# berkeley-hipie/HIPIE

Measured on AMD Instinct MI355X. Metric: images/sec @1024x1024 ViT-H bs=8 (single-image inference hot path: box, class and mask logits), higher is better.
Workload: dtype f16x3 (split-fp16 operands, fp32 accumulate: fp32-class); 1 GPU; BASELINE.json configs[2]: vit_huge, 1024x1024, batch 8 per GPU, 80 class prompts (L=194), detection; global_batch=8, parallelism=dp1, precision_policy=split, launch=eager

## Files before the change

### hipie_amd/csrc/gemm.hip

```cpp
#include "gemm_tile.h"

namespace hipie {

template <typename T>
__global__ __launch_bounds__(256) void to_hl8_kernel(const T* __restrict__ x, f16_t* __restrict__ out, long rows, int K, long ldx, long ldo,
                                                     float scale) {
  const long gid = (long)blockIdx.x * 256 + threadIdx.x;
  const int gpr = K / 8;
  if (gid >= rows * gpr) return;
  const long r = gid / gpr;
  const int g = (int)(gid - r * gpr);
  const T* src = x + r * ldx + 8 * g;
  f16x8 h, l;
#pragma unroll
  for (int e = 0; e < 8; ++e) {
    f16_t hh, ll;
    hl_split((float)src[e] * scale, hh, ll);
    h[e] = hh;
    l[e] = ll;
  }
  f16_t* dst = out + r * ldo + 16 * g;
  *reinterpret_cast<f16x8*>(dst) = h;
  *reinterpret_cast<f16x8*>(dst + 8) = l;
}
// ... 23 lines not shown
  __syncthreads();
  for (int u = tid; u < kTrCols * (kTrRows / 8); u += 256) {
    const int g = u % (kTrRows / 8), c = u / (kTrRows / 8);
    const long m = r0 + 8 * g;
    if (c0 + c >= C || m >= rows_p) continue;
    f16x8 h, l;
#pragma unroll
    for (int e = 0; e < 8; ++e) {
      f16_t hh, ll;
      hl_split(tile[8 * g + e][c] * scale, hh, ll);
      h[e] = hh;
      l[e] = ll;
    }
    f16_t* dst = out + (long)(c0 + c) * ldo + 2 * m;
    *reinterpret_cast<f16x8*>(dst) = h;
    *reinterpret_cast<f16x8*>(dst + 8) = l;
  }
}

}

using namespace hipie;

namespace hipie {
int launch_gemm_k256(const void* X, long ldx_b, int x_f32, const void* W, long ldw_b, const float* bias, float* out, long ldo, int M, int N,
                     hipStream_t st);
}

static inline bool gemm_mfma16() {
  const char* e = study_env("HIPIE_GEMM_MFMA");
  return e ? atoi(e) == 16 : true;
}

static int gemm_impl(const void* A, int64_t lda, const void* W, int64_t ldw, const float* bias, const float* resid, int64_t ldr,
                     void* out, int64_t ldo, const int32_t* out_row, const int32_t* a_row, int64_t a_rows, int M, int N, int K, int in_fmt,
                     int out_fmt, int act, float alpha, float oscale, void* stream, const float* alpha_dev = nullptr) {
  HIPIE_REQUIRE(A && W && out, "gemm: null pointer");
  HIPIE_REQUIRE(in_fmt == HIPIE_F16 || in_fmt == HIPIE_HL8 || in_fmt == HIPIE_F32, "gemm: operand format %d (HIPIE_F16 | HIPIE_HL8 | HIPIE_F32)",
                in_fmt);
  HIPIE_REQUIRE(out_fmt == HIPIE_F32 || out_fmt == HIPIE_F16 || out_fmt == HIPIE_HL8, "gemm: output format %d", out_fmt);
  HIPIE_REQUIRE(act >= 0 && act <= 3, "gemm: activation %d (0 none, 1 gelu, 2 relu, 3 quick-gelu)", act);
  HIPIE_REQUIRE(M > 0 && N > 0 && K > 0 && N % 8 == 0, "gemm: M=%d N=%d K=%d (N must be a multiple of 8)", M, N, K);
  const bool a_f32 = in_fmt == HIPIE_F32;
  const bool split = in_fmt == HIPIE_HL8 || a_f32;
  if (a_f32) lda *= 2;
  const int kq = split ? 32 : 64;
  HIPIE_REQUIRE(K % kq == 0, "gemm: K=%d must be a multiple of %d", K, kq);
  const int epr = split ? 2 * K : K;
  HIPIE_TRY(gm_check_operands("gemm", lda, ldw, epr, 320));
  HIPIE_TRY(gm_check_out("gemm", ldo, out_fmt, N));
  HIPIE_TRY(gm_check_resid("gemm", resid, ldr, N));
  HIPIE_TRY(gm_check_aligned("gemm", {A, W, out, bias, resid}));
  GemmParams p;
  gm_set_operands(p, A, lda, W, ldw, M, N, K, kq);
  p.bias = bias; p.resid = resid; p.ldr = ldr; p.out = (char*)out; p.ldo = ldo; p.out_row = out_row; p.a_row = a_row;
  p.out_fmt = out_fmt; p.act = act; p.alpha = alpha; p.oscale = oscale; p.alpha_dev = alpha_dev;
  hipStream_t st = (hipStream_t)stream;
  static const int k256_mode = [] { const char* e = study_env("HIPIE_GEMM_K256"); return e ? atoi(e) : 2; }();
  const bool k256_on = k256_mode == 1 || (k256_mode == 2 && N >= 384);
  if (k256_on && split && K == 256 && out_fmt == HIPIE_F32 && act == 0 && resid == nullptr && out_row == nullptr && a_row == nullptr &&
      alpha == 1.f && oscale == 1.f && alpha_dev == nullptr && N % 32 == 0 && M >= 8192 && ldw * 2 == 1024 && (long)M * p.lda_b < (1L << 32))
    return launch_gemm_k256(A, p.lda_b, a_f32 ? 1 : 0, W, p.ldw_b, bias, (float*)out, ldo, M, N, st);
  const bool wide = (N % 320 == 0);
  static const int small_on = [] { const char* e = study_env("HIPIE_GEMM_SMALL"); return e ? atoi(e) : 1; }();
  static const long small_tiles = [] { const char* e = study_env("HIPIE_GEMM_SMALL_MAXTILES"); return e ? atol(e) : 96L; }();
  const bool small_ok = small_on && (long)((M + 255) / 256) * ((N + (wide ? 319 : 255)) / (wide ? 320 : 256)) < small_tiles;
#ifdef HIPIE_GEMM_VARIANTS
  { const char* e = study_env("HIPIE_GEMM_VARIANT"); const int v = e ? atoi(e) : 0;
    if (split && wide && v == 1) return launch_gemm<320, true, 1>(p, st);
    if (split && wide && v == 3) return launch_gemm<320, true, 3>(p, st); }
  { const char* e = study_env("HIPIE_GEMM_VARIANT"); if (e) p.variant = atoi(e); }
  p.prio_mode = gemm2_prio();
  if (split && gemm2_mode() == 4) {
    const bool w160 = (N % 160 == 0);
    if (a_f32) return w160 ? launch_gemm4<5, 2>(p, st) : launch_gemm4<4, 2>(p, st);
    return w160 ? launch_gemm4<5, 0>(p, st) : launch_gemm4<4, 0>(p, st);
  }
  if (split && gemm2_mode() == 2) {
    const bool w160 = (N % 160 == 0);
    if (a_f32) return w160 ? launch_gemm3<5, 2>(p, st) : launch_gemm3<4, 2>(p, st);
    return w160 ? launch_gemm3<5, 0>(p, st) : launch_gemm3<4, 0>(p, st);
  }
  if (split && gemm2_mode() == 1) {
    const bool w160 = (N % 160 == 0);
    if (a_f32) return w160 ? launch_gemm2<5, 2>(p, st) : launch_gemm2<4, 2>(p, st);
    return w160 ? launch_gemm2<5, 0>(p, st) : launch_gemm2<4, 0>(p, st);
  }
#endif
  if (split && small_ok && a_row == nullptr) return a_f32 ? launch_gemm_small<2>(p, st) : launch_gemm_small<0>(p, st);
  if (split && wide && gemm_mfma16()) return a_f32 ? launch_gemm<320, true, 2, 16>(p, st) : launch_gemm<320, true, 0, 16>(p, st);
  if (a_f32) return wide ? launch_gemm<320, true, 2>(p, st) : launch_gemm<256, true, 2>(p, st);
  if (split) return wide ? launch_gemm<320, true>(p, st) : launch_gemm<256, true>(p, st);
  return wide ? launch_gemm<320, false>(p, st) : launch_gemm<256, false>(p, st);
}

extern "C" int hipie_gemm(const void* A, int64_t lda, const void* W, int64_t ldw, const float* bias, const float* resid, int64_t ldr,
                          void* out, int64_t ldo, const int32_t* out_row, int M, int N, int K, int in_fmt, int out_fmt, int act, float alpha,
                          float oscale, void* stream) {
  return gemm_impl(A, lda, W, ldw, bias, resid, ldr, out, ldo, out_row, nullptr, 0, M, N, K, in_fmt, out_fmt, act, alpha, oscale, stream);
}

extern "C" int hipie_gemm_scaled(const void* A, int64_t lda, const void* W, int64_t ldw, const float* bias, const float* resid, int64_t ldr,
                                 void* out, int64_t ldo, const int32_t* out_row, int M, int N, int K, int in_fmt, int out_fmt, int act, float alpha,
                                 float oscale, const float* alpha_dev, void* stream) {
  HIPIE_REQUIRE(((uintptr_t)alpha_dev % 4) == 0, "gemm_scaled: alpha_dev must be 4-byte aligned");
  return gemm_impl(A, lda, W, ldw, bias, resid, ldr, out, ldo, out_row, nullptr, 0, M, N, K, in_fmt, out_fmt, act, alpha, oscale, stream, alpha_dev);
}

extern "C" int hipie_gemm_gather(const void* A, int64_t lda, int64_t a_rows, const int32_t* a_row, const void* W, int64_t ldw, const float* bias,
                                 const float* resid, int64_t ldr, void* out, int64_t ldo, const int32_t* out_row, int M, int N, int K, int in_fmt,
                                 int out_fmt, int act, float alpha, float oscale, void* stream) {
  HIPIE_REQUIRE(a_row != nullptr && a_rows > 0, "gemm_gather: a_row map / operand row count missing");
  HIPIE_REQUIRE(in_fmt == HIPIE_HL8 || in_fmt == HIPIE_F32, "gemm_gather: split operands only (HIPIE_HL8 | HIPIE_F32 rows)");
  HIPIE_REQUIRE((long)a_rows * lda * (in_fmt == HIPIE_F32 ? 4 : 2) < (1L << 32), "gemm_gather: the gathered operand must stay below 4 GiB");
  return gemm_impl(A, lda, W, ldw, bias, resid, ldr, out, ldo, out_row, a_row, a_rows, M, N, K, in_fmt, out_fmt, act, alpha, oscale, stream);
}

extern "C" int hipie_gemm_batched(const void* A, int64_t lda, int64_t a_outer, int64_t a_inner, const void* W, int64_t ldw, int64_t w_outer,
                                  int64_t w_inner, void* out, int64_t ldo, int64_t o_outer, int64_t o_inner, int n_outer, int n_inner, int M,
                                  int N, int K, int out_fmt, float alpha, void* stream) {
  HIPIE_REQUIRE(A && W && out, "gemm_batched: null pointer");
  HIPIE_REQUIRE(out_fmt == HIPIE_F32 || out_fmt == HIPIE_HL8, "gemm_batched: output format %d (HIPIE_F32 | HIPIE_HL8)", out_fmt);
  HIPIE_REQUIRE(M > 0 && N > 0 && K > 0 && N % 8 == 0 && K % 32 == 0, "gemm_batched: M=%d N=%d K=%d (N %% 8, K %% 32)", M, N, K);
// ... 126 lines not shown
```

### hipie_amd/csrc/gemm_k256.hip

```cpp
#include <stdlib.h>

#include "common.h"
#include "mfma.h"
#include "wave.h"

namespace hipie {

struct TKParams {
  const char* X; const char* W; const float* bias; float* out;
  long ldx_b, ldw_b, ldo;
  int M, N;
};

constexpr int TK_K = 256, TK_C = 32;
constexpr int TK_TILE = TK_C * TK_K * 4;

template <bool XF32>
__global__ __launch_bounds__(256, 2) void gemm_k256_kernel(const TKParams p) {
  typedef f16_t T;
  typedef Mfma32<T>::frag frag;
  constexpr int KS = TK_K / 16;
  extern __shared__ __attribute__((aligned(1024))) char smem[];

  const int tid = threadIdx.x, lane = tid & 63;
  const int wave = __builtin_amdgcn_readfirstlane(tid >> 6);
  const int li = lane & 31, hi = lane >> 5;
  const int m = blockIdx.x * 128 + wave * 32 + li;
  const int mc = min(m, p.M - 1);
  const int nch = p.N / TK_C;

  unsigned int dv[8];
#pragma unroll
  for (int q = 0; q < 8; ++q) {
    const int i = wave + 4 * q;
    dv[q] = (unsigned int)((long)i * p.ldw_b + 16 * (lane ^ (i & 15)));
  }
  const unsigned int lds0 = (unsigned int)reinterpret_cast<uintptr_t>((__attribute__((address_space(3))) char*)smem);
  auto dma_chunk = [&](const int c, const int buf, const int q) __attribute__((always_inline)) {
    const int i = wave + 4 * q;
    dma16(p.W + (long)c * TK_C * p.ldw_b, dv[q], __builtin_amdgcn_readfirstlane(lds0 + (unsigned int)(buf * TK_TILE + 1024 * i)));
  };

  frag xh[KS], xl[KS];
  {
    const int m0w = blockIdx.x * 128 + wave * 32;
    const unsigned int xslice = lds0 + (unsigned int)(wave * 16384);
    const char* xs = smem + wave * 16384 + li * 512;
    unsigned int xv[16];
#pragma unroll
    for (int j = 0; j < 16; ++j) {
// ... 9 lines not shown
#pragma unroll
      for (int ksl = 0; ksl < KS / 2; ++ksl) {
        const int ks = half * (KS / 2) + ksl;
        const int u = 2 * (2 * ksl + hi);
        const frag a = *reinterpret_cast<const frag*>(xs + 16 * (u ^ (li & 15)));
        const frag b = *reinterpret_cast<const frag*>(xs + 16 * ((u + 1) ^ (li & 15)));
        if (XF32) {
          const f32x4 fa = __builtin_bit_cast(f32x4, a), fb = __builtin_bit_cast(f32x4, b);
          const float v[8] = {fa[0], fa[1], fa[2], fa[3], fb[0], fb[1], fb[2], fb[3]};
#pragma unroll
          for (int e = 0; e < 8; ++e) {
            T h, l;
            hl_split(v[e], h, l);
            xh[ks][e] = h;
            xl[ks][e] = l;
          }
        } else {
          xh[ks] = a;
          xl[ks] = b;
        }
      }
    }
    __builtin_amdgcn_s_waitcnt(lgkmcnt0);
    __syncthreads();
  }
#pragma unroll
  for (int q = 0; q < 8; ++q) dma_chunk(0, 0, q);

  const int wrow = li * 1024, wsw = li & 15;
  float* orow = p.out + (long)mc * p.ldo + 4 * hi;
  float4 prev[4];
#pragma unroll
  for (int g = 0; g < 4; ++g) prev[g] = make_float4(0.f, 0.f, 0.f, 0.f);

  for (int c = 0; c < nch; ++c) {
    const int buf = c & 1;
    __builtin_amdgcn_s_waitcnt(vmcnt(0));
    __syncthreads();
    if (c > 0 && m < p.M) {
#pragma unroll
      for (int g = 0; g < 4; ++g) *reinterpret_cast<float4*>(orow + 32 * (c - 1) + 8 * g) = prev[g];
    }
    const char* bs = smem + buf * TK_TILE;
    const bool more = c + 1 < nch;
    f32x16 h0, h1;
#pragma unroll
    for (int r = 0; r < 16; ++r) { h0[r] = 0.f; h1[r] = 0.f; }
#pragma unroll
    for (int ks = 0; ks < KS; ks += 2) {
      const frag ah0 = *reinterpret_cast<const frag*>(bs + wrow + 16 * ((2 * (2 * ks + hi)) ^ wsw));
      const frag al0 = *reinterpret_cast<const frag*>(bs + wrow + 16 * ((2 * (2 * ks + hi) + 1) ^ wsw));
      const frag ah1 = *reinterpret_cast<const frag*>(bs + wrow + 16 * ((2 * (2 * ks + 2 + hi)) ^ wsw));
      const frag al1 = *reinterpret_cast<const frag*>(bs + wrow + 16 * ((2 * (2 * ks + 2 + hi) + 1) ^ wsw));
      h0 = Mfma32<T>::mma(al0, xh[ks], h0);
      h1 = Mfma32<T>::mma(al1, xh[ks + 1], h1);
      h0 = Mfma32<T>::mma(ah0, xl[ks], h0);
      h1 = Mfma32<T>::mma(ah1, xl[ks + 1], h1);
      h0 = Mfma32<T>::mma(ah0, xh[ks], h0);
      h1 = Mfma32<T>::mma(ah1, xh[ks + 1], h1);
      if (more) dma_chunk(c + 1, buf ^ 1, ks >> 1);
    }
#pragma unroll
    for (int g = 0; g < 4; ++g) {
      float4 b4 = make_float4(0.f, 0.f, 0.f, 0.f);
      if (p.bias) b4 = *reinterpret_cast<const float4*>(p.bias + 32 * c + 8 * g + 4 * hi);
      prev[g] = make_float4(h0[4 * g] + h1[4 * g] + b4.x, h0[4 * g + 1] + h1[4 * g + 1] + b4.y, h0[4 * g + 2] + h1[4 * g + 2] + b4.z,
                            h0[4 * g + 3] + h1[4 * g + 3] + b4.w);
    }
  }
  if (m < p.M) {
#pragma unroll
    for (int g = 0; g < 4; ++g) *reinterpret_cast<float4*>(orow + 32 * (nch - 1) + 8 * g) = prev[g];
  }
}

int launch_gemm_k256(const void* X, long ldx_b, int x_f32, const void* W, long ldw_b, const float* bias, float* out, long ldo, int M, int N,
                     hipStream_t st) {
  TKParams p;
  p.X = (const char*)X; p.W = (const char*)W; p.bias = bias; p.out = out;
  p.ldx_b = ldx_b; p.ldw_b = ldw_b; p.ldo = ldo;
  p.M = M; p.N = N;
  const size_t lds = (size_t)2 * TK_TILE;
  static LdsLimit limit[2];
  limit[0].raise((const void*)gemm_k256_kernel<true>, lds);
  limit[1].raise((const void*)gemm_k256_kernel<false>, lds);
  const dim3 grid((unsigned)((M + 127) / 128));
  if (x_f32) hipLaunchKernelGGL(gemm_k256_kernel<true>, grid, dim3(256), lds, st, p);
  else hipLaunchKernelGGL(gemm_k256_kernel<false>, grid, dim3(256), lds, st, p);
  return check_launch("gemm_k256");
}

}
```

### hipie_amd/csrc/gemm_tile.h

```cpp
#pragma once
#include <stdlib.h>

#include <initializer_list>

#include "common.h"
#include "gelu.h"
#include "mfma.h"
#include "wave.h"

namespace hipie {

struct GemmParams {
  const char* A = nullptr; const char* W = nullptr; const float* bias = nullptr; const float* resid = nullptr; char* out = nullptr;
  const int32_t* out_row = nullptr;
  const int32_t* a_row = nullptr;
  long lda_b = 0, ldw_b = 0;
  long ldr = 0, ldo = 0;
  int M = 0, N = 0, K = 0;
  int nkt = 0;
  int tiles_m = 0, tiles_n = 0;
  int group_m = 0;
  int out_fmt = HIPIE_F32, act = 0;
  float alpha = 1.f, oscale = 1.f;
  int nbi = 1;
// ... 98 lines not shown
                           __builtin_bit_cast(unsigned int, v[g][2]), __builtin_bit_cast(unsigned int, v[g][3])};
    } else {
#pragma unroll
      for (int g = 0; g < NG; ++g) {
        unsigned int H0, L0, H1, L1;
        gm_split2(v[g][0], v[g][1], H0, L0);
        gm_split2(v[g][2], v[g][3], H1, L1);
#if defined(__HIP_DEVICE_COMPILE__) && !defined(HIPIE_NO_FMA_MIX)
        asm volatile("s_nop 1" : "+v"(H0), "+v"(L0), "+v"(H1), "+v"(L1));
#endif
        const u32x2 s0 = __builtin_amdgcn_permlane32_swap(H0, L0, false, false);
        const u32x2 s1 = __builtin_amdgcn_permlane32_swap(H1, L1, false, false);
        piece[g] = (u32x4){s0[0], s1[0], s0[1], s1[1]};
      }
    }
    const long rowb = (m * p.ldo) * (ofmt == HIPIE_F32 ? 4 : 2) + (long)nb * 4 + 16 * hi;
#pragma unroll
    for (int g = 0; g < NG; ++g)
      if (mok && nb + 8 * (G0 + g) < p.N) *reinterpret_cast<u32x4*>(p.out + rowb + 32 * (G0 + g)) = piece[g];
  }
}

template <int G0, int NG>
__device__ __forceinline__ void gm_epi_quads(const f32x16& a, const float4* rq, const float* sb, const long m, const bool mok, const int nb,
                                             const int hi, const GemmParams& p, const bool has_res) {
  float x[NG][4];
#pragma unroll
  for (int g = 0; g < NG; ++g)
#pragma unroll
    for (int e = 0; e < 4; ++e) x[g][e] = a[4 * (G0 + g) + e];
  gm_epi_vals<NG>(x, G0, rq, sb, m, mok, nb, hi, p, has_res);
}

__device__ __forceinline__ constexpr int gm_swz16(const int r) { return ((r >> 1) & 3) | (((((r & 15) + 4) >> 3) & 1) << 2); }

__device__ __forceinline__ void gm_epi_vals16(const float (&x)[2][4], const float4* rq, const float* sb, const long m, const bool mok, const int nb,
                                              const int g, const GemmParams& p, const bool has_res) {
  typedef unsigned int u32x2 __attribute__((ext_vector_type(2)));
  typedef unsigned int u32x4 __attribute__((ext_vector_type(4)));
  const float alpha = p.alpha, osc = p.oscale;
  const int act = p.act, ofmt = p.out_fmt;
  float v[2][4];
#pragma unroll
  for (int i = 0; i < 2; ++i) {
    const float4 b4 = *reinterpret_cast<const float4*>(sb + 16 * i + 4 * g);
    v[i][0] = x[i][0] * alpha + b4.x;
    v[i][1] = x[i][1] * alpha + b4.y;
    v[i][2] = x[i][2] * alpha + b4.z;
    v[i][3] = x[i][3] * alpha + b4.w;
  }
  if (act == 1) {
#pragma unroll
    for (int i = 0; i < 2; ++i)
#pragma unroll
      for (int e = 0; e < 4; ++e) v[i][e] = gm_gelu(v[i][e]);
  } else if (act == 2) {
#pragma unroll
    for (int i = 0; i < 2; ++i)
#pragma unroll
      for (int e = 0; e < 4; ++e) v[i][e] = fmaxf(v[i][e], 0.f);
  } else if (act == 3) {
#pragma unroll
    for (int i = 0; i < 2; ++i)
#pragma unroll
      for (int e = 0; e < 4; ++e) v[i][e] = v[i][e] / (1.f + expf(-1.702f * v[i][e]));
  }
// ... 127 lines not shown
#pragma unroll
  for (int t = 0; t < NT; ++t) {
    const int m = m0 + wm * 64 + t * 16 + c;
    orow[t] = (m < p.M) ? (p.out_row != nullptr ? (long)p.out_row[m] : (long)m) : -1;
  }
  float4 rq[2][2];
  auto load_res = [&](const int blk, float4 (&dst)[2]) {
    const int t = blk / (NF / 2), jp = blk % (NF / 2);
#pragma unroll
    for (int i = 0; i < 2; ++i) {
      const int n = n0 + wn * (BN / 2) + jp * 32 + 16 * i + 4 * g;
      dst[i] = (has_res && orow[t] >= 0 && n < p.N) ? *reinterpret_cast<const float4*>(p.resid + orow[t] * p.ldr + n) : make_float4(0.f, 0.f, 0.f, 0.f);
    }
  };
  load_res(0, rq[0]);
#pragma unroll
  for (int t = 0; t < NT; ++t) {
    const long m = orow[t];
#pragma unroll
    for (int jp = 0; jp < NF / 2; ++jp) {
      const int blk = t * (NF / 2) + jp;
      if (blk + 1 < NT * (NF / 2)) load_res(blk + 1, rq[(blk + 1) & 1]);
      const int nb = n0 + wn * (BN / 2) + jp * 32;
      float x[2][4];
#pragma unroll
      for (int i = 0; i < 2; ++i)
#pragma unroll
        for (int e = 0; e < 4; ++e) x[i][e] = acc[2 * jp + i][t][e];
      gm_epi_vals16(x, rq[blk & 1], sbias + (nb - n0), m, m >= 0, nb, g, p, has_res);
    }
  }
}

template <int BN, bool SPLIT, int VAR, int MS = 32>
__global__ __launch_bounds__(512, 2) void gemm_kernel(const GemmParams pin) {
  static_assert(MS == 32 || (MS == 16 && BN == 320 && SPLIT && (VAR == 0 || VAR == 2)),
                "the 16x16x32 form exists for the wide split instances (HL8 and fp32 A rows) only");
  GemmParams p = pin;
  gm_alpha_dev(p);
  int vtile = -1;
  if (VAR == 8) {
    const int nblk = p.tiles_m * p.tiles_n * p.nbi;
    const int id = blockIdx.x, xcd = id & 7, j = id >> 3;
    const int q = nblk >> 3, r = nblk & 7;
    const int v = (xcd < r ? xcd * (q + 1) : r * (q + 1) + (xcd - r) * q) + j;
    const int bo = blockIdx.y, bi = v % p.nbi;
    vtile = v / p.nbi;
    p.A += bo * p.a_bo + bi * p.a_bi;
    p.W += bo * p.w_bo + bi * p.w_bi;
    p.out += bo * p.o_bo + bi * p.o_bi;
    if (p.sm_mask != nullptr) p.sm_mask += (long)bo * p.sm_L;
    if (p.sm_bias != nullptr) p.sm_bias += ((long)bo * p.nbi + bi) * p.N;
  } else if (gridDim.y > 1) {
    const int bo = blockIdx.y / p.nbi, bi = blockIdx.y - bo * p.nbi;
    p.A += bo * p.a_bo + bi * p.a_bi;
    p.W += bo * p.w_bo + bi * p.w_bi;
    p.out += bo * p.o_bo + bi * p.o_bi;
    if (p.sm_mask != nullptr) p.sm_mask += (long)bo * p.sm_L;
    if (p.sm_bias != nullptr) p.sm_bias += (long)blockIdx.y * p.N;
    if (p.resid != nullptr) p.resid += bo * p.r_bo + bi * p.r_bi;
  }
  constexpr int BM = 256;
  constexpr int ROWS = BM + BN;
  constexpr int STAGE = ROWS * 128;
  constexpr int NI = ROWS / 64;
  constexpr int NJ = BN / 64;
  constexpr int KS = SPLIT ? 2 : 4;
  constexpr int SUB = KS * NJ;
  constexpr bool AF32 = VAR == 2 || VAR == 6;
  constexpr bool LNE = VAR == 4 || VAR == 6;
// ... 104 lines not shown
      if (SPLIT) wa[s & 1][1] = *reinterpret_cast<const frag*>(ws + j * 4096 + choff(ks, 1));
    };
    load_x(0);
    load_w(0);
    constexpr int DMA_BY = SPLIT ? 4 : 6;
    constexpr int PER = (NI + DMA_BY - 1) / DMA_BY;
    frag cx[2][2];
#pragma unroll
    for (int s = 0; s < SUB; ++s) {
      const int ks = s / NJ, j = s % NJ;
      if (s + 1 < SUB) {
        if ((s + 1) % NJ == 0) load_x(ks + 1);
        load_w(s + 1);
      }
      if (AF32 && j == 0) {
#pragma unroll
        for (int t = 0; t < 2; ++t) {
          const f32x4 a = __builtin_bit_cast(f32x4, xa[ks & 1][0][t]), b = __builtin_bit_cast(f32x4, xa[ks & 1][1][t]);
#pragma unroll
          for (int e = 0; e < 4; ++e) {
            f16_t hh, ll;
            hl_split(a[e], hh, ll);
            cx[0][t][e] = hh; cx[1][t][e] = ll;
            hl_split(b[e], hh, ll);
            cx[0][t][4 + e] = hh; cx[1][t][4 + e] = ll;
          }
        }
      }
      const frag wh = wa[s & 1][0];
      const frag xh0 = AF32 ? cx[0][0] : xa[ks & 1][0][0], xh1 = AF32 ? cx[0][1] : xa[ks & 1][0][1];
      if (SPLIT) {
        const frag wl = wa[s & 1][1];
        const frag xl0 = AF32 ? cx[1][0] : xa[ks & 1][1][0], xl1 = AF32 ? cx[1][1] : xa[ks & 1][1][1];
        acc[j][0] = Mfma32<f16_t>::mma(wl, xh0, acc[j][0]);
        acc[j][1] = Mfma32<f16_t>::mma(wl, xh1, acc[j][1]);
        acc[j][0] = Mfma32<f16_t>::mma(wh, xl0, acc[j][0]);
        acc[j][1] = Mfma32<f16_t>::mma(wh, xl1, acc[j][1]);
      }
      acc[j][0] = Mfma32<f16_t>::mma(wh, xh0, acc[j][0]);
      acc[j][1] = Mfma32<f16_t>::mma(wh, xh1, acc[j][1]);
      if (more) {
#pragma unroll
        for (int i = s * PER; i < (s + 1) * PER && i < NI; ++i) dma(i, kt + 1, st ^ 1);
      }
    }
    __builtin_amdgcn_s_waitcnt(vmcnt(0));
    __syncthreads();
  }

  bool has_res = p.resid != nullptr;
#ifdef HIPIE_GEMM_VARIANTS
  if (VAR == 1 && p.alpha != 12345.f) return;
#endif
  const int act = p.act, ofmt = p.out_fmt;
  const float alpha = p.alpha, osc = p.oscale;
  float* sbias = reinterpret_cast<float*>(smem);
  if (tid < BN) sbias[tid] = (p.bias != nullptr && n0 + tid < p.N) ? p.bias[n0 + tid] : 0.f;
  if (SPLIT && LNE && BN == 256) {
    float* lg = sbias + 256;
    float* lb = lg + 256;
    float* red = lb + 256;
    if (tid < 256) { lg[tid] = p.ln_g[tid]; lb[tid] = p.ln_b[tid]; }
    __syncthreads();
    float su[2] = {0.f, 0.f};
    f32x4 rr[2][4];
    auto ln_res = [&](const int blk, f32x4 (&dst)[4]) {
      const int t = blk / NJ, j = blk % NJ;
      const int m = min(m0 + wm * 64 + t * 32 + li, p.M - 1);
#pragma unroll
      for (int g = 0; g < 4; ++g) {
        const int n = wn * (BN / 2) + j * 32 + 8 * g + 4 * hi;
        dst[g] = *reinterpret_cast<const f32x4*>(p.resid + (long)m * p.ldr + n);
      }
// ... 34 lines not shown
      for (int j = 0; j < NJ; ++j)
#pragma unroll
        for (int r = 0; r < 16; ++r) { const float d = acc[j][t][r] - mean[t]; q += d * d; }
      sq[t] = q + __shfl_xor(q, 32);
    }
    __syncthreads();
#pragma unroll
    for (int t = 0; t < 2; ++t)
      if (hi == 0) red[wn * 256 + wm * 64 + t * 32 + li] = sq[t];
    __syncthreads();
    float rstd[2];
#pragma unroll
    for (int t = 0; t < 2; ++t) rstd[t] = rsqrtf((sq[t] + red[(wn ^ 1) * 256 + wm * 64 + t * 32 + li]) / 256.f + p.ln_eps);
#pragma unroll
    for (int j = 0; j < NJ; ++j) {
#pragma unroll
      for (int t = 0; t < 2; ++t)
#pragma unroll
        for (int g = 0; g < 4; ++g) {
          const int n = wn * (BN / 2) + j * 32 + 8 * g + 4 * hi;
          const f32x4 g4 = *reinterpret_cast<const f32x4*>(lg + n), b4 = *reinterpret_cast<const f32x4*>(lb + n);
#pragma unroll
          for (int e = 0; e < 4; ++e) acc[j][t][4 * g + e] = (acc[j][t][4 * g + e] - mean[t]) * rstd[t] * g4[e] + b4[e];
        }
#if defined(__HIP_DEVICE_COMPILE__)
      __builtin_amdgcn_sched_barrier(0);
#endif
    }
    __syncthreads();
    if (tid < BN) sbias[tid] = 0.f;
    p.alpha = 1.f; p.act = 0; p.oscale = 1.f; p.out_fmt = HIPIE_F32;
    has_res = false;
  }
  if (SPLIT && (VAR == 0 || VAR == 8) && BN == 256 && p.softmax) {
    float* kb = sbias + 256;
    float* red = kb + 256;
    float* cb = red + 512;
    if (tid < 256) kb[tid] = (tid < p.sm_L && (p.sm_mask == nullptr || p.sm_mask[tid] != 0)) ? 0.f : -INFINITY;
    if (VAR == 8 && tid < 256) cb[tid] = (p.sm_bias != nullptr && tid < p.N) ? p.sm_bias[tid] : 0.f;
    __syncthreads();
    const float cl = p.sm_clamp;
    float mx[2] = {-INFINITY, -INFINITY};
#pragma unroll
    for (int t = 0; t < 2; ++t)
#pragma unroll
      for (int j = 0; j < NJ; ++j)
#pragma unroll
        for (int g = 0; g < 4; ++g) {
          const f32x4 k4 = *reinterpret_cast<const f32x4*>(kb + wn * (BN / 2) + j * 32 + 8 * g + 4 * hi);
          f32x4 c4 = {0.f, 0.f, 0.f, 0.f};
          if (VAR == 8) c4 = *reinterpret_cast<const f32x4*>(cb + wn * (BN / 2) + j * 32 + 8 * g + 4 * hi);
#pragma unroll
          for (int e = 0; e < 4; ++e) {
            float x = acc[j][t][4 * g + e] * p.alpha;
            if (VAR == 8) x += c4[e];
            if (cl > 0.f) x = __builtin_amdgcn_fmed3f(x, -cl, cl);
            x += k4[e];
            acc[j][t][4 * g + e] = x;
            mx[t] = fmaxf(mx[t], x);
          }
        }
#pragma unroll
    for (int t = 0; t < 2; ++t) {
      mx[t] = fmaxf(mx[t], __shfl_xor(mx[t], 32));
      if (hi == 0) red[wn * 256 + wm * 64 + t * 32 + li] = mx[t];
    }
    __syncthreads();
    float sm[2];
#pragma unroll
    for (int t = 0; t < 2; ++t) {
      const float m = fmaxf(mx[t], red[(wn ^ 1) * 256 + wm * 64 + t * 32 + li]);
      const float m2 = (m == -INFINITY) ? 0.f : m * 1.4426950408889634f;
      float su = 0.f;
#pragma unroll
      for (int j = 0; j < NJ; ++j)
#pragma unroll
        for (int r = 0; r < 16; ++r) {
          const float pv = __builtin_amdgcn_exp2f(acc[j][t][r] * 1.4426950408889634f - m2);
          acc[j][t][r] = pv;
          su += pv;
        }
      sm[t] = su + __shfl_xor(su, 32);
    }
    __syncthreads();
#pragma unroll
    for (int t = 0; t < 2; ++t)
      if (hi == 0) red[wn * 256 + wm * 64 + t * 32 + li] = sm[t];
    __syncthreads();
#pragma unroll
    for (int t = 0; t < 2; ++t) {
      const float tot = sm[t] + red[(wn ^ 1) * 256 + wm * 64 + t * 32 + li];
      const float inv = tot > 0.f ? 1.f / tot : 0.f;
#pragma unroll
      for (int j = 0; j < NJ; ++j)
#pragma unroll
        for (int r = 0; r < 16; ++r) acc[j][t][r] *= inv;
    }
    p.alpha = 1.f;
  }
  __syncthreads();
  float4 rq[2][4];
  long orow[2];
#pragma unroll
  for (int t = 0; t < 2; ++t) {
    const int m = m0 + wm * 64 + t * 32 + li;
    orow[t] = (m < p.M) ? (p.out_row != nullptr ? (long)p.out_row[m] : (long)m) : -1;
  }
  auto load_res = [&](const int t, const int j, float4 (&dst)[4]) {
#pragma unroll
    for (int g = 0; g < 4; ++g) {
      const int n = n0 + wn * (BN / 2) + j * 32 + 8 * g + 4 * hi;
      dst[g] = (has_res && orow[t] >= 0 && n < p.N) ? *reinterpret_cast<const float4*>(p.resid + orow[t] * p.ldr + n) : make_float4(0.f, 0.f, 0.f, 0.f);
    }
  };
  const int passes = (LNE && p.out2 != nullptr) ? 2 : 1;
#pragma unroll
  for (int pass = 0; pass < 2; ++pass) {
    if (pass >= passes) break;
    if (pass == 1) { p.out = p.out2; p.ldo = p.ldo2; p.out_fmt = HIPIE_HL8; }
    load_res(0, 0, rq[0]);
#pragma unroll
    for (int t = 0; t < 2; ++t) {
      const long m = orow[t];
      const bool mok = m >= 0;
#pragma unroll
      for (int j = 0; j < NJ; ++j) {
        const int blk = t * NJ + j;
        if (blk + 1 < 2 * NJ) load_res((blk + 1) / NJ, (blk + 1) % NJ, rq[(blk + 1) & 1]);
        const int nb = n0 + wn * (BN / 2) + j * 32;
        gm_epi_quads<0, 4>(acc[j][t], rq[blk & 1], sbias + (nb - n0), m, mok, nb, hi, p, has_res);
#if defined(__HIP_DEVICE_COMPILE__)
        if (LNE) __builtin_amdgcn_sched_barrier(0);
#endif
// ... 103 lines not shown
  if (tid < BN) sbias[tid] = (p.bias != nullptr && n0 + tid < p.N) ? p.bias[n0 + tid] : 0.f;
  __syncthreads();
  const int nb = n0 + wave * 32;
#pragma unroll
  for (int t = 0; t < 2; ++t) {
    const int mm = m0 + t * 32 + li;
    const long m = (mm < p.M) ? (p.out_row != nullptr ? (long)p.out_row[mm] : (long)mm) : -1;
    float4 rq[4];
#pragma unroll
    for (int g = 0; g < 4; ++g) {
      const int n = nb + 8 * g + 4 * hi;
      rq[g] = (has_res && m >= 0 && n < p.N) ? *reinterpret_cast<const float4*>(p.resid + m * p.ldr + n) : make_float4(0.f, 0.f, 0.f, 0.f);
    }
    gm_epi_quads<0, 4>(acc[t], rq, sbias + wave * 32, m, m >= 0, nb, hi, p, has_res);
  }
}

template <int VAR>
static int launch_gemm_small(GemmParams& p, hipStream_t st) {
  constexpr size_t lds = (size_t)3 * (64 + 128) * 128;
  p.tiles_m = (p.M + 63) / 64;
  p.tiles_n = (p.N + 127) / 128;
  auto kern = gemm_small_kernel<VAR>;
  static LdsLimit limit;
  limit.raise((const void*)kern, lds);
  hipLaunchKernelGGL(kern, dim3((unsigned)(p.tiles_m * p.tiles_n)), dim3(256), lds, st, p);
  return check_launch("gemm_small");
}

#ifdef HIPIE_GEMM_VARIANTS
#include "../../tools/ubench/gemm_overlap_study.h"
#endif

template <int BN, bool SPLIT, int VAR = 0, int MS = 32>
static int launch_gemm(GemmParams& p, hipStream_t st, int batches = 1) {
  constexpr size_t lds = (size_t)2 * (256 + BN) * 128;
  p.tiles_m = (p.M + 255) / 256;
  p.tiles_n = (p.N + BN - 1) / BN;
  p.group_m = p.tiles_n > 4 ? 8 : 0;
  auto kern = gemm_kernel<BN, SPLIT, VAR, MS>;
  static LdsLimit limit;
  limit.raise((const void*)kern, lds);
  if (VAR == 8)
    hipLaunchKernelGGL(kern, dim3((unsigned)(p.tiles_m * p.tiles_n * p.nbi), (unsigned)(batches / p.nbi)), dim3(512), lds, st, p);
  else
    hipLaunchKernelGGL(kern, dim3((unsigned)(p.tiles_m * p.tiles_n), (unsigned)batches), dim3(512), lds, st, p);
  return check_launch("gemm");
}

static inline void gm_set_operands(GemmParams& p, const void* A, long lda, const void* W, long ldw, int M, int N, int K, int kq = 32) {
  p.A = (const char*)A; p.W = (const char*)W;
  p.lda_b = lda * 2; p.ldw_b = ldw * 2;
  p.M = M; p.N = N; p.K = K; p.nkt = K / kq;
}

static inline void gm_set_batch(GemmParams& p, int n_inner, long a_outer, long a_inner, long w_outer, long w_inner, long o_outer, long o_inner,
                                long osz) {
  p.nbi = n_inner;
  p.a_bo = a_outer * 2; p.a_bi = a_inner * 2; p.w_bo = w_outer * 2; p.w_bi = w_inner * 2; p.o_bo = o_outer * osz; p.o_bi = o_inner * osz;
}

static inline int gm_check_operands(const char* who, long lda, long ldw, int epr, int bn) {
  if (!(lda >= epr && ldw >= epr && lda % 8 == 0 && ldw % 8 == 0))
    return set_err(HIPIE_EINVAL, "%s: operand row strides %ld / %ld (>= %d, multiples of 8)", who, lda, ldw, epr);
  if (!(256 * lda * 2 < (1L << 31) && bn * ldw * 2 < (1L << 31))) return set_err(HIPIE_EINVAL, "%s: row stride too large", who);
  return 0;
}

static inline int gm_check_out(const char* who, long ldo, int out_fmt, int N) {
  const int opr = out_fmt == HIPIE_HL8 ? 2 * N : N;
  if (!(ldo >= opr && ldo % 4 == 0)) return set_err(HIPIE_EINVAL, "%s: output row stride %ld (>= %d)", who, ldo, opr);
  return 0;
}
// ... 25 lines not shown
```

### hipie_amd/csrc/wave.h

```cpp
#pragma once
#include "common.h"

namespace hipie {

__device__ __forceinline__ void dma16(const char* sbase, unsigned int voff, unsigned int lds_dst) {
#if defined(__HIP_DEVICE_COMPILE__)
  unsigned int keep;
  asm volatile("s_mov_b32 %0, m0\n\ts_mov_b32 m0, %3\n\ts_nop 0\n\tglobal_load_lds_dwordx4 %1, %2\n\ts_mov_b32 m0, %0"
               : "=&s"(keep) : "v"(voff), "s"(sbase), "s"(lds_dst) : "memory");
#endif
}

__device__ __forceinline__ void dma16_off(const void* gsrc, unsigned int lds_dst) {
#if defined(__HIP_DEVICE_COMPILE__)
  unsigned int keep;
  asm volatile("s_mov_b32 %0, m0\n\ts_mov_b32 m0, %2\n\ts_nop 0\n\tglobal_load_lds_dwordx4 %1, off\n\ts_mov_b32 m0, %0"
               : "=&s"(keep) : "v"(gsrc), "s"(lds_dst) : "memory");
#endif
}

__device__ __forceinline__ void dma16_masked(const char* sbase, unsigned int voff, unsigned int lds_dst, unsigned long long mask) {
#if defined(__HIP_DEVICE_COMPILE__)
  unsigned long long save;
  asm volatile("s_and_saveexec_b64 %0, %4\n\ts_mov_b32 m0, %3\n\ts_nop 0\n\tglobal_load_lds_dwordx4 %1, %2\n\ts_mov_b64 exec, %0"
               : "=&s"(save) : "v"(voff), "s"(sbase), "s"(lds_dst), "s"(mask) : "memory", "m0");
#endif
}

constexpr int vmcnt(int n) { return 0x0F70 | (n & 15) | ((n >> 4) << 14); }
constexpr int lgkmcnt0 = 0xC07F;

__device__ __forceinline__ float max3(float a, float b, float c) {
  float d;
  asm("v_max3_f32 %0, %1, %2, %3" : "=v"(d) : "v"(a), "v"(b), "v"(c));
  return d;
}

__device__ __forceinline__ float xhalf_max(float x) {
  typedef unsigned int u32x2 __attribute__((ext_vector_type(2)));
  const unsigned int u = __builtin_bit_cast(unsigned int, x);
  const u32x2 r = __builtin_amdgcn_permlane32_swap(u, u, false, false);
  return fmaxf(__builtin_bit_cast(float, (unsigned int)r[0]), __builtin_bit_cast(float, (unsigned int)r[1]));
}

__device__ __forceinline__ float wave_max(float x) {
#pragma unroll
  for (int o = 32; o > 0; o >>= 1) x = fmaxf(x, __shfl_xor(x, o));
  return x;
}

__device__ __forceinline__ float wave_sum(float x) {
#pragma unroll
  for (int o = 32; o > 0; o >>= 1) x += __shfl_xor(x, o);
  return x;
}
__device__ __forceinline__ double wave_sum(double x) {
#pragma unroll
  for (int o = 32; o > 0; o >>= 1) x += __shfl_xor(x, o);
  return x;
// ... 71 lines not shown
```

Baseline: 43.32 images/sec.

## Transpose MFMA accumulator to store fp32 output rows directly in GEMM epilogues

Swaps the MFMA operand order so each lane's accumulator holds a column and its registers run across output rows. Lanes then write consecutive columns of the same row, giving coalesced scalar-base fp32 stores without the LDS or float4 staging step. This applies to the K=256 kernel and to a new 256-column split GEMM path used when K<=256, fp32 output and no residual. The cost is 16 narrow dword stores per fragment instead of float4 stores, a separate masked epilogue, and a new ldo limit so offsets fit in 32 bits.

```diff
diff --git a/hipie_amd/csrc/gemm.hip b/hipie_amd/csrc/gemm.hip
--- a/hipie_amd/csrc/gemm.hip
+++ b/hipie_amd/csrc/gemm.hip
@@ -79,6 +79,11 @@
   return e ? atoi(e) == 16 : true;
 }
 
+static inline bool gemm_rowspan(const int K) {
+  const char* e = study_env("HIPIE_GEMM_ROWSPAN");
+  return e ? atoi(e) != 0 : K <= 256;
+}
+
 static int gemm_impl(const void* A, int64_t lda, const void* W, int64_t ldw, const float* bias, const float* resid, int64_t ldr,
                      void* out, int64_t ldo, const int32_t* out_row, const int32_t* a_row, int64_t a_rows, int M, int N, int K, int in_fmt,
                      int out_fmt, int act, float alpha, float oscale, void* stream, const float* alpha_dev = nullptr) {
@@ -106,7 +111,7 @@
   static const int k256_mode = [] { const char* e = study_env("HIPIE_GEMM_K256"); return e ? atoi(e) : 2; }();
   const bool k256_on = k256_mode == 1 || (k256_mode == 2 && N >= 384);
   if (k256_on && split && K == 256 && out_fmt == HIPIE_F32 && act == 0 && resid == nullptr && out_row == nullptr && a_row == nullptr &&
-      alpha == 1.f && oscale == 1.f && alpha_dev == nullptr && N % 32 == 0 && M >= 8192 && ldw * 2 == 1024 && (long)M * p.lda_b < (1L << 32))
+      alpha == 1.f && oscale == 1.f && alpha_dev == nullptr && N % 32 == 0 && M >= 8192 && ldw * 2 == 1024 && (long)M * p.lda_b < (1L << 32) && ldo < (1L << 24))
     return launch_gemm_k256(A, p.lda_b, a_f32 ? 1 : 0, W, p.ldw_b, bias, (float*)out, ldo, M, N, st);
   const bool wide = (N % 320 == 0);
   static const int small_on = [] { const char* e = study_env("HIPIE_GEMM_SMALL"); return e ? atoi(e) : 1; }();
@@ -134,8 +139,10 @@
     return w160 ? launch_gemm2<5, 0>(p, st) : launch_gemm2<4, 0>(p, st);
   }
 #endif
+  const bool rows = split && out_fmt == HIPIE_F32 && resid == nullptr && ldo < (1L << 24) && gemm_rowspan(K);
   if (split && small_ok && a_row == nullptr) return a_f32 ? launch_gemm_small<2>(p, st) : launch_gemm_small<0>(p, st);
   if (split && wide && gemm_mfma16()) return a_f32 ? launch_gemm<320, true, 2, 16>(p, st) : launch_gemm<320, true, 0, 16>(p, st);
+  if (rows && !wide) return a_f32 ? launch_gemm<256, true, 2, 32, true>(p, st) : launch_gemm<256, true, 0, 32, true>(p, st);
   if (a_f32) return wide ? launch_gemm<320, true, 2>(p, st) : launch_gemm<256, true, 2>(p, st);
   if (split) return wide ? launch_gemm<320, true>(p, st) : launch_gemm<256, true>(p, st);
   return wide ? launch_gemm<320, false>(p, st) : launch_gemm<256, false>(p, st);
diff --git a/hipie_amd/csrc/gemm_k256.hip b/hipie_amd/csrc/gemm_k256.hip
--- a/hipie_amd/csrc/gemm_k256.hip
+++ b/hipie_amd/csrc/gemm_k256.hip
@@ -15,7 +15,7 @@
 constexpr int TK_K = 256, TK_C = 32;
 constexpr int TK_TILE = TK_C * TK_K * 4;
 
-template <bool XF32>
+template <bool XF32, bool ROWS>
 __global__ __launch_bounds__(256, 2) void gemm_k256_kernel(const TKParams p) {
   typedef f16_t T;
   typedef Mfma32<T>::frag frag;
@@ -91,12 +91,31 @@
   float4 prev[4];
 #pragma unroll
   for (int g = 0; g < 4; ++g) prev[g] = make_float4(0.f, 0.f, 0.f, 0.f);
+  const int m0w = blockIdx.x * 128 + wave * 32;
+  const unsigned int olane = (unsigned int)(4 * (4 * hi * (int)p.ldo + li));
+  const int rows_ok = p.M - m0w - 4 * hi;
+  float prow[16];
+#pragma unroll
+  for (int r = 0; r < 16; ++r) prow[r] = 0.f;
+  auto store_rows = [&](const int c) __attribute__((always_inline)) {
+    char* const ob = reinterpret_cast<char*>(p.out + (long)m0w * p.ldo + 32 * c);
+    if (m0w + 32 <= p.M) {
+#pragma unroll
+      for (int r = 0; r < 16; ++r) store_f32_ubase(ob + 4 * crow(r, 0) * p.ldo, olane, prow[r]);
+    } else {
+#pragma unroll
+      for (int r = 0; r < 16; ++r)
+        if (crow(r, 0) < rows_ok) store_f32_ubase(ob + 4 * crow(r, 0) * p.ldo, olane, prow[r]);
+    }
+  };
 
   for (int c = 0; c < nch; ++c) {
     const int buf = c & 1;
     __builtin_amdgcn_s_waitcnt(vmcnt(0));
     __syncthreads();
-    if (c > 0 && m < p.M) {
+    if (ROWS) {
+      if (c > 0) store_rows(c - 1);
+    } else if (c > 0 && m < p.M) {
 #pragma unroll
       for (int g = 0; g < 4; ++g) *reinterpret_cast<float4*>(orow + 32 * (c - 1) + 8 * g) = prev[g];
     }
@@ -111,13 +130,28 @@
       const frag al0 = *reinterpret_cast<const frag*>(bs + wrow + 16 * ((2 * (2 * ks + hi) + 1) ^ wsw));
       const frag ah1 = *reinterpret_cast<const frag*>(bs + wrow + 16 * ((2 * (2 * ks + 2 + hi)) ^ wsw));
       const frag al1 = *reinterpret_cast<const frag*>(bs + wrow + 16 * ((2 * (2 * ks + 2 + hi) + 1) ^ wsw));
-      h0 = Mfma32<T>::mma(al0, xh[ks], h0);
-      h1 = Mfma32<T>::mma(al1, xh[ks + 1], h1);
-      h0 = Mfma32<T>::mma(ah0, xl[ks], h0);
-      h1 = Mfma32<T>::mma(ah1, xl[ks + 1], h1);
-      h0 = Mfma32<T>::mma(ah0, xh[ks], h0);
-      h1 = Mfma32<T>::mma(ah1, xh[ks + 1], h1);
+      if (ROWS) {
+        h0 = Mfma32<T>::mma(xh[ks], al0, h0);
+        h1 = Mfma32<T>::mma(xh[ks + 1], al1, h1);
+        h0 = Mfma32<T>::mma(xl[ks], ah0, h0);
+        h1 = Mfma32<T>::mma(xl[ks + 1], ah1, h1);
+        h0 = Mfma32<T>::mma(xh[ks], ah0, h0);
+        h1 = Mfma32<T>::mma(xh[ks + 1], ah1, h1);
+      } else {
+        h0 = Mfma32<T>::mma(al0, xh[ks], h0);
+        h1 = Mfma32<T>::mma(al1, xh[ks + 1], h1);
+        h0 = Mfma32<T>::mma(ah0, xl[ks], h0);
+        h1 = Mfma32<T>::mma(ah1, xl[ks + 1], h1);
+        h0 = Mfma32<T>::mma(ah0, xh[ks], h0);
+        h1 = Mfma32<T>::mma(ah1, xh[ks + 1], h1);
+      }
       if (more) dma_chunk(c + 1, buf ^ 1, ks >> 1);
+    }
+    if (ROWS) {
+      const float bv = p.bias ? p.bias[32 * c + li] : 0.f;
+#pragma unroll
+      for (int r = 0; r < 16; ++r) prow[r] = h0[r] + h1[r] + bv;
+      continue;
     }
 #pragma unroll
     for (int g = 0; g < 4; ++g) {
@@ -127,10 +161,17 @@
                             h0[4 * g + 3] + h1[4 * g + 3] + b4.w);
     }
   }
-  if (m < p.M) {
+  if (ROWS) {
+    store_rows(nch - 1);
+  } else if (m < p.M) {
 #pragma unroll
     for (int g = 0; g < 4; ++g) *reinterpret_cast<float4*>(orow + 32 * (nch - 1) + 8 * g) = prev[g];
   }
+}
+
+static inline bool k256_rowspan() {
+  const char* e = study_env("HIPIE_GEMM_ROWSPAN");
+  return e ? atoi(e) != 0 : true;
 }
 
 int launch_gemm_k256(const void* X, long ldx_b, int x_f32, const void* W, long ldw_b, const float* bias, float* out, long ldo, int M, int N,
@@ -140,12 +181,19 @@
   p.ldx_b = ldx_b; p.ldw_b = ldw_b; p.ldo = ldo;
   p.M = M; p.N = N;
   const size_t lds = (size_t)2 * TK_TILE;
-  static LdsLimit limit[2];
-  limit[0].raise((const void*)gemm_k256_kernel<true>, lds);
-  limit[1].raise((const void*)gemm_k256_kernel<false>, lds);
+  static LdsLimit limit[4];
+  limit[0].raise((const void*)gemm_k256_kernel<true, false>, lds);
+  limit[1].raise((const void*)gemm_k256_kernel<false, false>, lds);
+  limit[2].raise((const void*)gemm_k256_kernel<true, true>, lds);
+  limit[3].raise((const void*)gemm_k256_kernel<false, true>, lds);
   const dim3 grid((unsigned)((M + 127) / 128));
-  if (x_f32) hipLaunchKernelGGL(gemm_k256_kernel<true>, grid, dim3(256), lds, st, p);
-  else hipLaunchKernelGGL(gemm_k256_kernel<false>, grid, dim3(256), lds, st, p);
+  if (k256_rowspan()) {
+    if (x_f32) hipLaunchKernelGGL((gemm_k256_kernel<true, true>), grid, dim3(256), lds, st, p);
+    else hipLaunchKernelGGL((gemm_k256_kernel<false, true>), grid, dim3(256), lds, st, p);
+  } else {
+    if (x_f32) hipLaunchKernelGGL((gemm_k256_kernel<true, false>), grid, dim3(256), lds, st, p);
+    else hipLaunchKernelGGL((gemm_k256_kernel<false, false>), grid, dim3(256), lds, st, p);
+  }
   return check_launch("gemm_k256");
 }
 
diff --git a/hipie_amd/csrc/gemm_tile.h b/hipie_amd/csrc/gemm_tile.h
--- a/hipie_amd/csrc/gemm_tile.h
+++ b/hipie_amd/csrc/gemm_tile.h
@@ -154,6 +154,59 @@
   gm_epi_vals<NG>(x, G0, rq, sb, m, mok, nb, hi, p, has_res);
 }
 
+__device__ __forceinline__ void gm_rows_vals(float (&v)[16], const f32x16& x, const float bv, const GemmParams& p) {
+  const float alpha = p.alpha, osc = p.oscale;
+  const int act = p.act;
+#pragma unroll
+  for (int r = 0; r < 16; ++r) v[r] = x[r] * alpha + bv;
+  if (act == 1) {
+#pragma unroll
+    for (int r = 0; r < 16; ++r) v[r] = gm_gelu(v[r]);
+  } else if (act == 2) {
+#pragma unroll
+    for (int r = 0; r < 16; ++r) v[r] = fmaxf(v[r], 0.f);
+  } else if (act == 3) {
+#pragma unroll
+    for (int r = 0; r < 16; ++r) v[r] = v[r] / (1.f + expf(-1.702f * v[r]));
+  }
+  if (osc != 1.f) {
+#pragma unroll
+    for (int r = 0; r < 16; ++r) v[r] *= osc;
+  }
+}
+
+__device__ __forceinline__ void gm_epi_rows_full(const f32x16& x, const float bv, const int mb, const int nb, const unsigned int olane, const GemmParams& p) {
+  float v[16];
+  gm_rows_vals(v, x, bv, p);
+  char* ob = p.out + 4 * ((long)mb * p.ldo + nb);
+  unsigned int ld4 = 4u * (unsigned int)p.ldo;
+#if defined(__HIP_DEVICE_COMPILE__)
+  asm volatile("" : "+s"(ld4));
+#endif
+#pragma unroll
+  for (int r = 0; r < 16; ++r) *reinterpret_cast<float*>(ob + (olane + crow(r, 0) * ld4)) = v[r];
+}
+
+__device__ __forceinline__ void gm_epi_rows_masked(const f32x16& x, const float bv, const int mb, const int n, const int hi, const GemmParams& p) {
+  const bool nok = n < p.N;
+  int orow[16];
+  int hil = hi;
+#if defined(__HIP_DEVICE_COMPILE__)
+  asm volatile("" : "+v"(hil));
+#endif
+#pragma unroll
+  for (int r = 0; r < 16; ++r) {
+    const int m = mb + crow(r, hil);
+    orow[r] = (m < p.M) ? (p.out_row != nullptr ? p.out_row[m] : m) : -1;
+  }
+  float v[16];
+  gm_rows_vals(v, x, bv, p);
+  float* const out = reinterpret_cast<float*>(p.out) + n;
+#pragma unroll
+  for (int r = 0; r < 16; ++r)
+    if (nok && orow[r] >= 0) out[(long)orow[r] * p.ldo] = v[r];
+}
+
 __device__ __forceinline__ constexpr int gm_swz16(const int r) { return ((r >> 1) & 3) | (((((r & 15) + 4) >> 3) & 1) << 2); }
 
 __device__ __forceinline__ void gm_epi_vals16(const float (&x)[2][4], const float4* rq, const float* sb, const long m, const bool mok, const int nb,
@@ -347,10 +400,12 @@
   }
 }
 
-template <int BN, bool SPLIT, int VAR, int MS = 32>
+template <int BN, bool SPLIT, int VAR, int MS = 32, bool TR = false>
 __global__ __launch_bounds__(512, 2) void gemm_kernel(const GemmParams pin) {
   static_assert(MS == 32 || (MS == 16 && BN == 320 && SPLIT && (VAR == 0 || VAR == 2)),
                 "the 16x16x32 form exists for the wide split instances (HL8 and fp32 A rows) only");
+  static_assert(!TR || (MS == 32 && BN == 256 && SPLIT && (VAR == 0 || VAR == 2)),
+                "the transposed accumulator (fp32 output, no residual: gm_epi_rows_full / _masked) exists for the 256-column split instances only");
   GemmParams p = pin;
   gm_alpha_dev(p);
   int vtile = -1;
@@ -521,13 +576,13 @@
       if (SPLIT) {
         const frag wl = wa[s & 1][1];
         const frag xl0 = AF32 ? cx[1][0] : xa[ks & 1][1][0], xl1 = AF32 ? cx[1][1] : xa[ks & 1][1][1];
-        acc[j][0] = Mfma32<f16_t>::mma(wl, xh0, acc[j][0]);
-        acc[j][1] = Mfma32<f16_t>::mma(wl, xh1, acc[j][1]);
-        acc[j][0] = Mfma32<f16_t>::mma(wh, xl0, acc[j][0]);
-        acc[j][1] = Mfma32<f16_t>::mma(wh, xl1, acc[j][1]);
-      }
-      acc[j][0] = Mfma32<f16_t>::mma(wh, xh0, acc[j][0]);
-      acc[j][1] = Mfma32<f16_t>::mma(wh, xh1, acc[j][1]);
+        acc[j][0] = TR ? Mfma32<f16_t>::mma(xh0, wl, acc[j][0]) : Mfma32<f16_t>::mma(wl, xh0, acc[j][0]);
+        acc[j][1] = TR ? Mfma32<f16_t>::mma(xh1, wl, acc[j][1]) : Mfma32<f16_t>::mma(wl, xh1, acc[j][1]);
+        acc[j][0] = TR ? Mfma32<f16_t>::mma(xl0, wh, acc[j][0]) : Mfma32<f16_t>::mma(wh, xl0, acc[j][0]);
+        acc[j][1] = TR ? Mfma32<f16_t>::mma(xl1, wh, acc[j][1]) : Mfma32<f16_t>::mma(wh, xl1, acc[j][1]);
+      }
+      acc[j][0] = TR ? Mfma32<f16_t>::mma(xh0, wh, acc[j][0]) : Mfma32<f16_t>::mma(wh, xh0, acc[j][0]);
+      acc[j][1] = TR ? Mfma32<f16_t>::mma(xh1, wh, acc[j][1]) : Mfma32<f16_t>::mma(wh, xh1, acc[j][1]);
       if (more) {
 #pragma unroll
         for (int i = s * PER; i < (s + 1) * PER && i < NI; ++i) dma(i, kt + 1, st ^ 1);
@@ -628,7 +683,7 @@
     p.alpha = 1.f; p.act = 0; p.oscale = 1.f; p.out_fmt = HIPIE_F32;
     has_res = false;
   }
-  if (SPLIT && (VAR == 0 || VAR == 8) && BN == 256 && p.softmax) {
+  if (!TR && SPLIT && (VAR == 0 || VAR == 8) && BN == 256 && p.softmax) {
     float* kb = sbias + 256;
     float* red = kb + 256;
     float* cb = red + 512;
@@ -695,6 +750,30 @@
     p.alpha = 1.f;
   }
   __syncthreads();
+  if constexpr (TR) {
+    float bv[NJ];
+#pragma unroll
+    for (int j = 0; j < NJ; ++j) bv[j] = sbias[wn * (BN / 2) + j * 32 + li];
+    const int mw = m0 + wm * 64, nw = n0 + wn * (BN / 2);
+    if (p.out_row == nullptr && m0 + BM <= p.M && n0 + BN <= p.N) {
+      const unsigned int olane = (unsigned int)(4 * (4 * hi * (int)p.ldo + li));
+#pragma unroll
+      for (int t = 0; t < 2; ++t)
+#pragma unroll
+        for (int j = 0; j < NJ; ++j) gm_epi_rows_full(acc[j][t], bv[j], mw + 32 * t, nw + 32 * j, olane, p);
+    } else {
+#pragma unroll
+      for (int t = 0; t < 2; ++t)
+#pragma unroll
+        for (int j = 0; j < NJ; ++j) {
+          gm_epi_rows_masked(acc[j][t], bv[j], mw + 32 * t, nw + 32 * j + li, hi, p);
+#if defined(__HIP_DEVICE_COMPILE__)
+          __builtin_amdgcn_sched_barrier(0);
+#endif
+        }
+    }
+    return;
+  }
   float4 rq[2][4];
   long orow[2];
 #pragma unroll
@@ -864,13 +943,13 @@
 #include "../../tools/ubench/gemm_overlap_study.h"
 #endif
 
-template <int BN, bool SPLIT, int VAR = 0, int MS = 32>
+template <int BN, bool SPLIT, int VAR = 0, int MS = 32, bool TR = false>
 static int launch_gemm(GemmParams& p, hipStream_t st, int batches = 1) {
   constexpr size_t lds = (size_t)2 * (256 + BN) * 128;
   p.tiles_m = (p.M + 255) / 256;
   p.tiles_n = (p.N + BN - 1) / BN;
   p.group_m = p.tiles_n > 4 ? 8 : 0;
-  auto kern = gemm_kernel<BN, SPLIT, VAR, MS>;
+  auto kern = gemm_kernel<BN, SPLIT, VAR, MS, TR>;
   static LdsLimit limit;
   limit.raise((const void*)kern, lds);
   if (VAR == 8)
diff --git a/hipie_amd/csrc/wave.h b/hipie_amd/csrc/wave.h
--- a/hipie_amd/csrc/wave.h
+++ b/hipie_amd/csrc/wave.h
@@ -25,6 +25,13 @@
   asm volatile("s_and_saveexec_b64 %0, %4\n\ts_mov_b32 m0, %3\n\ts_nop 0\n\tglobal_load_lds_dwordx4 %1, %2\n\ts_mov_b64 exec, %0"
                : "=&s"(save) : "v"(voff), "s"(sbase), "s"(lds_dst), "s"(mask) : "memory", "m0");
 #endif
+}
+
+__device__ __forceinline__ void store_f32_ubase(char* base, unsigned int voff, float v) {
+  typedef __attribute__((address_space(1))) float gfloat;
+  const unsigned long long u = reinterpret_cast<unsigned long long>(base);
+  const unsigned int lo = __builtin_amdgcn_readfirstlane((unsigned int)u), hi = __builtin_amdgcn_readfirstlane((unsigned int)(u >> 32));
+  *reinterpret_cast<gfloat*>((((unsigned long long)hi << 32) | lo) + voff) = v;
 }
 
 constexpr int vmcnt(int n) { return 0x0F70 | (n & 15) | ((n >> 4) << 14); }
```

New measurement: 43.07 images/sec. About the same (-0.6%).
